# fgvieira/ngsF-HMM

Measured on AMD Instinct MI355X. Metric: site-ind updates/sec (EM iterations x individuals x sites / s), 1M sites x 1k ind, higher is better.
Workload: dtype f64

## Files before the change

ngsf-hmm_amd/csrc/kernels_fast.hip:

```cpp
#include <hip/hip_runtime.h>

#include "fast_dev.hpp"

namespace nghmm {

namespace {


__global__ void __launch_bounds__(256)
k_fast_geno_interleave(const uint32_t* __restrict__ codes, uint64_t cell0, uint64_t I, uint64_t S,
                       uint64_t T, uint32_t C, uint32_t* __restrict__ geno_il) {
  const uint64_t TB = T >> 4;
  const uint64_t n = I * C * TB * 64;
  for (uint64_t k = (uint64_t)blockIdx.x * blockDim.x + threadIdx.x; k < n;
       k += (uint64_t)gridDim.x * blockDim.x) {
    const uint64_t lane = k & 63, r = k >> 6;
    const uint64_t tb = r % TB, wv = r / TB;
    const uint64_t c = wv % C, i = wv / C;
    const uint64_t s0 = (c * 64 + lane) * T + tb * 16;
    uint32_t w = 0;
#pragma unroll
    for (int j = 0; j < 16; ++j) {
      const uint64_t s = s0 + j;
      if (s < S) w |= gl_code(codes, cell0 + s * I + i) << (2 * j);
// ... 150 lines not shown
      const uint32_t code = (w >> ((uint32_t)(t & 15) * 2)) & 3u;
      const double u = arr.u_lin;
      const double u0 = fma(u, h00, fma(u, 2 * bb, u * h02));
      const double u1 = fma(u, h00 + bb, u * (h02 + bb));
      e0 = code == 0 ? h00 : code == 1 ? 2 * bb : code == 2 ? h02 : u0;
      e1 = code == 0 ? h00 + bb : code == 1 ? 0.0 : code == 2 ? h02 + bb : u1;
    } else {
      const double* g = gl_lin + (s * I + i) * 3;
      e0 = fma(g[0], h00, fma(g[1], 2 * bb, g[2] * h02));
      e1 = fma(g[0], h00 + bb, g[2] * (h02 + bb));
    }
    out[k * 2] = log(e0);
    out[k * 2 + 1] = log(e1);
  }
}

struct SwitchName {
  const char* name;
  int Switches::*field;
};
const SwitchName kSwitches[] = {
    {"bg_parts", &Switches::bg_parts}, {"estmaf_interp", &Switches::estmaf_interp},
    {"estmaf_no_rows", &Switches::estmaf_no_rows}, {"estmaf_no_called", &Switches::estmaf_no_called},
    {"fast_c", &Switches::fast_c}, {"exact_serial", &Switches::exact_serial},
    {"dbg_abort_round", &Switches::dbg_abort_round}, {"no_dev_bfgs", &Switches::no_dev_bfgs},
    {"no_bg_stream", &Switches::no_bg_stream}, {"spans", &Switches::spans},
    {"viterbi_chunk", &Switches::viterbi_chunk}};

}

Switches Switches::from_env() {
  Switches sw;
  for (const auto& k : kSwitches) {
    std::string env = "NGHMM_";
    for (const char* c = k.name; *c; ++c) env += (char)std::toupper((unsigned char)*c);
    if (const char* v = std::getenv(env.c_str())) {
      char* end = nullptr;
      const long n = std::strtol(v, &end, 10);
      sw.*(k.field) = (end != v) ? (int)n : 1;
    }
  }
  return sw;
}

bool Switches::set(const char* name, long value) {
  for (const auto& k : kSwitches)
// ... 217 lines not shown
```

ngsf-hmm_amd/csrc/kernels_fast.hpp:

```cpp
#pragma once

#include <hip/hip_runtime.h>

#include <cstdint>
#include <map>
#include <vector>

#include "glview.hpp"

namespace nghmm {

struct Switches {
  int bg_parts = 2;
  int estmaf_interp = 1;
  int estmaf_no_rows = 0;
  int estmaf_no_called = 0;
  int fast_c = 0;
  int exact_serial = 0;
  int dbg_abort_round = 0;
  int no_dev_bfgs = 0;
  int no_bg_stream = 0;
  int viterbi_chunk = 0;
  int spans = 0;
  static Switches from_env();
  bool set(const char* name, long value);
};

struct SiteShard {
  uint32_t rank = 0, world = 1;
  double* send = nullptr;
  double* recv = nullptr;
  uint64_t cap = 0;
  int (*allgather)(void* user, uint64_t n_bytes) = nullptr;
  void* user = nullptr;
  double* edges = nullptr;
  bool edges_from_round = false;
  uint64_t n_gathers = 0;
};

// ... 58 lines not shown
    double *snap_F = nullptr, *snap_A = nullptr;
    uint32_t snap_set = 0;
    volatile uint32_t* h_table = nullptr;
    double *h_F = nullptr, *h_A = nullptr;
    unsigned long long stats_host[6] = {0, 0, 0, 0, 0, 0};
    uint32_t seq_base = 0;
    uint32_t mstep_no = 0;
    bool clean = true;
    bool preplanned = false;
    bool pre_F_fixed = false, pre_alpha_fixed = false;
    double* h_epi_lkl = nullptr;
    volatile uint32_t* h_epi = nullptr;
    uint32_t epi_seq = 0;
  } dev;

  double dmax_finite = 0;
  double alpha_small_min = 0;
  uint8_t* redo = nullptr;
  size_t redo_cap = 0;
  uint8_t* est_status = nullptr;
  double* est_state = nullptr;
  std::map<uint32_t, uint64_t> mode_ind_rounds;
  uint32_t* est_counts = nullptr;
};

enum EstCount {
  EST_CNT_CHECK_FAILED = 0,
  EST_CNT_RESUMED = 1,
  EST_CNT_RESUMED_AGAIN = 2,
  EST_CNT_LOGSPACE = 3,
  EST_CNT_EXACT_TAIL = 4,
  EST_COUNTS = 5
};

bool fast_create(FastState& fs, uint64_t I, uint64_t S, bool packed = false);
bool fast_create_replica(FastState& fs, const FastState& parent);
void fast_destroy(FastState& fs);
bool fast_load(FastState& fs, hipStream_t st, const GlView& gl_log, const double* d_pos);
bool fast_refresh_freq_table(FastState& fs, hipStream_t st, const double* d_freq, int* d_flags);
bool fast_refresh_emissions(FastState& fs, hipStream_t st, const double* d_freq, int* d_flags);
bool fast_lkl_prepare(FastState& fs, hipStream_t st, uint32_t n_pts, const uint32_t* h_ind,
                      const double* h_F, const double* h_A, bool force_general = false);
bool fast_lkl_launch(FastState& fs, hipStream_t st, double* d_lkl, int* d_flags,
                     bool emit_estep = false);
bool fast_lkl_covers_everyone(const FastState& fs);
bool dbfgs_available(const FastState& fs);
bool dbfgs_reserve(FastState& fs);
void dbfgs_destroy(FastState& fs);
void dbfgs_invalidate(FastState& fs);
constexpr uint32_t kEpiFlags = 8;
bool dbfgs_epilogue(FastState& fs, hipStream_t st, int* d_flags, uint32_t n_flags, const double* d_lkl);
bool dbfgs_wait_epilogue(FastState& fs, hipStream_t st, int* flags_out, uint32_t n_flags, bool yield);
bool dbfgs_begin(FastState& fs, hipStream_t st, double* d_indF, double* d_alpha, bool F_fixed,
                 bool alpha_fixed);
const double* dbfgs_start_F(const FastState& fs);
// ... 36 lines not shown
```

ngsf-hmm_amd/csrc/kernels_fast_estmaf.hip:

```cpp
#include "fast_dev.hpp"

#include <mutex>

namespace capi {
void set_error(const char* fmt, ...);
}

namespace nghmm {

namespace {



__device__ double2 estmaf_term_logspace(const double* g, double freq, double F) {
  double h[3];
  h[0] = (1 - freq) * (1 - freq) + (1 - freq) * freq * F;
  h[1] = 2 * (1 - freq) * freq - 2 * (1 - freq) * freq * F;
  h[2] = freq * freq + (1 - freq) * freq * F;
  double pp[3];
  for (int k = 0; k < 3; ++k) {
    double l = log(h[k]);
    if (l == -__builtin_huge_val()) l = -kINF;
    h[k] = l;
  }
// ... 69 lines not shown
    const int l = __builtin_amdgcn_update_dpp(0, (int)(uint32_t)b, 0x142, 0xa, 0xf, false);
    const int h = __builtin_amdgcn_update_dpp(0, (int)(uint32_t)(b >> 32), 0x142, 0xa, 0xf, false);
    v += ngh_from_bits(((uint64_t)(uint32_t)h << 32) | (uint32_t)l);
  }
  return v;
}

constexpr int EN = 12;
constexpr int EST_SCALARS = 8;
constexpr int EST_FIELDS = EST_SCALARS + 2 * EN;
enum : uint8_t { EST_DONE = 0, EST_INTERP = 1, EST_EXACT = 2 };
constexpr int EST_K0 = 2;
constexpr int EST_MIN_GAIN = 24;
constexpr double EST_DMAX = 0.85;
constexpr double EST_BACK = 0.1;
constexpr double EST_MULT = 32.0;
constexpr double EST_FIT = 0.72;
constexpr int EST_KMAX = 32;
constexpr double EST_TOL = 1e-11;
constexpr double EST_GUARD = 1e-9;
__constant__ double kChebC[EN] = {0.9914448613738104, 0.9238795325112867, 0.7933533402912352, 0.6087614290087207, 0.38268343236508984, 0.1305261922200517, -0.1305261922200516, -0.3826834323650895, -0.6087614290087207, -0.793353340291235, -0.9238795325112867, -0.9914448613738104};
__constant__ double kChebW[EN] = {0.13052619222005157, -0.3826834323650898, 0.6087614290087207, -0.7933533402912352, 0.9238795325112867, -0.9914448613738104, 0.9914448613738104, -0.9238795325112868, 0.7933533402912352, -0.6087614290087209, 0.3826834323650899, -0.130526192220052};

constexpr int ESTMAF_MAXW = 16;

__device__ __forceinline__ bool in_tile_rows(uint64_t site, uint64_t tile_T, uint64_t row0,
                                             uint64_t row1) {
  if (tile_T == 0) return true;
  const uint64_t j = site / tile_T, t = site - j * tile_T;
  const uint64_t row = (j >> 6) * tile_T + t;
  return row >= row0 && row < row1;
}
__host__ __device__ constexpr int estmaf_full_slots(int NI, int BLOCK) {
  return BLOCK == 64 ? (NI == 16 ? 12 : NI == 12 ? 8 : NI == 8 ? 4 : NI == 4 ? 2 : NI == 2 ? 1 : 0)
                     : (NI == 16 ? 8 : 0);
}

template <int NI, int BLOCK, bool TILE>
__device__ __forceinline__ void estmaf_site(
    const GlView& gl, const double* __restrict__ marg_blocks, uint64_t S_own, uint64_t I_tot,
    uint64_t I_blk, double* __restrict__ freq_out, uint8_t* __restrict__ redo,
    uint8_t* __restrict__ status, double* __restrict__ state, uint64_t state_stride, int fresh,
    int n_exact, int allow_build, uint64_t site, const double* __restrict__ tile_col,
    uint32_t* __restrict__ cnt, double (&xch)[2][ESTMAF_MAXW][2],
    double2 (&nodebuf)[(BLOCK == 64 && NI >= 8) ? EN : 1][(BLOCK == 64 && NI >= 8) ? 65 : 1],
    double2 (&xnode)[(BLOCK == 64 && NI >= 8) ? 1 : EN][(BLOCK == 64 && NI >= 8) ? 1 : BLOCK / 64],
    double2* park = nullptr) {
  constexpr int W = BLOCK / 64;
  constexpr bool PARK = (W == 1 && NI >= 8);
  const int lane = threadIdx.x & 63;
  const int wv = threadIdx.x >> 6;
  const uint32_t tix = threadIdx.x;
  constexpr uint64_t stride = BLOCK;
  const uint64_t cell_s = site * I_tot;

  double tF_lane_out;
  double sA[NI], sb[NI], sC[NI], u0[NI], nC[NI], fc[NI];
  {
    constexpr int NB = NI < 8 ? NI : (NI % 8 ? NI / 2 : 8);
    static_assert(NI % NB == 0, "whole batches");
    const bool one_block = (I_blk == I_tot);
    const uint32_t ib = (uint32_t)I_blk;
    double tF_acc = 0;
#pragma unroll
    for (int k0 = 0; k0 < NI; k0 += NB) {
      double r0[NB], r1[NB], r2[NB], rF[NB];
      uint64_t ic[NB];
// ... 254 lines not shown
                lane_sums(lane_value(r_nodes, nd), pn, pd);
                const double v = wave_sum_pair(pn, pd);
                const double sn = lane_value(v, 31), sd = lane_value(v, 63);
                if (lane == nd) {
                  an = sn;
                  ad = sd;
                }
              }
            }
            my_gn = an;
            my_gd = ad;
            check = true;
          }
        }
      }
    }
  }
  if (tix == 0) {
    const double freq = num / den;
    const bool ok = freq >= 0 && freq < 1;
    freq_out[site] = freq;
    redo[site] = ok ? 0 : 1;
    status[site] = EST_DONE;
  }
}

__device__ __forceinline__ const double* estmaf_tile_col(const double* marg_blocks, uint64_t site,
                                                         uint64_t tile_T, uint64_t I_tot) {
  const uint64_t j = site / tile_T, t = site - j * tile_T;
  return marg_blocks + post_lane_off((j >> 6) * tile_T + t, j & 63, I_tot);
}

#define ESTMAF_SHARED(NI, BLOCK)                                                              \
  constexpr bool PARK_ = ((BLOCK) == 64 && (NI) >= 8);                                         \
  __shared__ double xch[2][ESTMAF_MAXW][2];                       \
  __shared__ double2 nodebuf[PARK_ ? EN : 1][PARK_ ? 65 : 1];                                  \
  __shared__ double2 xnode[PARK_ ? 1 : EN][PARK_ ? 1 : (BLOCK) / 64]

template <int NI, int BLOCK, bool TILE>
__global__ void __launch_bounds__(BLOCK) __attribute__((amdgpu_waves_per_eu(2)))
k_fast_estmaf(const GlView gl, const double* __restrict__ marg_blocks,
              uint64_t S_own, uint64_t I_tot, uint64_t I_blk, uint64_t tile_T,
              double* __restrict__ freq_out, uint8_t* __restrict__ redo,
              uint8_t* __restrict__ status, double* __restrict__ state, uint64_t state_stride,
              int n_exact, int allow_build, uint64_t blk0, uint32_t* __restrict__ cnt) {
  ESTMAF_SHARED(NI, BLOCK);
  uint64_t site;
  const double* tile_col = nullptr;
  if constexpr (TILE) {
    const uint64_t b = blockIdx.x + blk0, x = b & 7, k = b >> 3;
    const uint64_t q = ((k >> 3) << 6) + (x << 3) + (k & 7);
    const uint64_t tile_row = q >> 6, l = q & 63;
    const uint64_t c = tile_row / tile_T, t = tile_row - c * tile_T;
    site = (c * 64 + l) * tile_T + t;
    if (site >= S_own) return;
    tile_col = marg_blocks + post_lane_off(tile_row, l, I_tot);
  } else {
    site = blockIdx.x;
  }
  extern __shared__ double2 park_mem[];
  estmaf_site<NI, BLOCK, TILE>(gl, marg_blocks, S_own, I_tot, I_blk, freq_out, redo, status, state,
                               state_stride, 1, n_exact, allow_build, site, tile_col, cnt, xch, nodebuf,
                               xnode, park_mem);
}

template <int NI, int BLOCK, bool TILE>
__global__ void __launch_bounds__(BLOCK) __attribute__((amdgpu_waves_per_eu(2)))
k_fast_estmaf_resume(const GlView gl, const double* __restrict__ marg_blocks,
                     uint64_t S_own, uint64_t I_tot, uint64_t I_blk, uint64_t tile_T,
                     double* __restrict__ freq_out, uint8_t* __restrict__ redo,
                     uint8_t* __restrict__ status, double* __restrict__ state,
                     uint64_t state_stride, int n_exact, int allow_build, uint64_t row0,
                     uint64_t row1, uint32_t* __restrict__ cnt, int cnt_slot) {
  ESTMAF_SHARED(NI, BLOCK);
  extern __shared__ double2 park_mem[];
  const int lane = threadIdx.x & 63;
  for (uint64_t base = (uint64_t)blockIdx.x * 64; base < S_own; base += (uint64_t)gridDim.x * 64) {
    const uint64_t s = base + lane;
    const bool need = s < S_own && in_tile_rows(s, TILE ? tile_T : 0, row0, row1) &&
                      status[s] == EST_EXACT;
    uint64_t mask = __ballot(need);
    if (mask && threadIdx.x == 0) atomicAdd(cnt + cnt_slot, (uint32_t)__popcll(mask));
    if constexpr (BLOCK > 64) __syncthreads();
    while (mask) {
      const uint64_t site = base + (uint64_t)__builtin_ctzll(mask);
      mask &= mask - 1;
      const double* tile_col = TILE ? estmaf_tile_col(marg_blocks, site, tile_T, I_tot) : nullptr;
      estmaf_site<NI, BLOCK, TILE>(gl, marg_blocks, S_own, I_tot, I_blk, freq_out, redo, status,
                                   state, state_stride, 0, n_exact, allow_build, site, tile_col, cnt,
                                   xch, nodebuf, xnode, park_mem);
      if constexpr (BLOCK > 64) __syncthreads();
    }
  }
}

__device__ __forceinline__ double row_sum(double v) {
  v = __dadd_rn(v, dpp_move<0xB1>(v));
  v = __dadd_rn(v, dpp_move<0x4E>(v));
  v = __dadd_rn(v, dpp_move<0x141>(v));
  v = __dadd_rn(v, dpp_move<0x140>(v));
  return v;
}

template <int NI, bool TILE>
__device__ __forceinline__ void estmaf_rows_sites(
    const GlView& gl, const double* __restrict__ marg_blocks, uint64_t S_own, uint64_t I_tot,
    uint64_t I_blk, double* __restrict__ freq_out, uint8_t* __restrict__ redo,
    uint8_t* __restrict__ status, double* __restrict__ state, uint64_t state_stride, int fresh,
    int n_exact, int allow_build, uint64_t site, const double* __restrict__ tile_col, bool done,
    uint32_t* __restrict__ cnt) {
  static_assert(EN <= 16, "a row's lanes hold the interval's node sums");
  const int lane = threadIdx.x, j = lane & 15;
  const uint64_t cell_s = site * I_tot;

  double sA[NI], sb[NI], sC[NI], u0[NI], nC[NI], fc[NI];
  double tF_acc = 0;
  {
    const bool one_block = (I_blk == I_tot);
    const uint32_t ib = (uint32_t)I_blk;
    double r0[NI], r1[NI], r2[NI], rF[NI];
    uint64_t ic[NI];
#pragma unroll
    for (int k = 0; k < NI; ++k) {
      const uint64_t i = (uint64_t)j + 16 * k;
      ic[k] = i < I_tot ? i : I_tot - 1;
      gl_fetch(gl, cell_s + ic[k], r0[k], r1[k], r2[k]);
    }
#pragma unroll
    for (int k = 0; k < NI; ++k) {
      if constexpr (TILE) {
        rF[k] = tile_col[post_ind_off(ic[k])];
      } else if (one_block) {
        rF[k] = marg_blocks[site * I_blk + ic[k]];
// ... 80 lines not shown
      const double bn = row_sum(q * my_gn) / Sq, bd = row_sum(q * my_gd) / Sq;
      if (check && !done) {
        interp_ok = fabs(bn - sn) <= EST_TOL * fabs(sn) && fabs(bd - sd) <= EST_TOL * fabs(sd);
        if (!interp_ok && j == 0) atomicAdd(cnt + EST_CNT_CHECK_FAILED, 1u);
      }
      check = false;
    }
    bool want_build = false;
    if (!done) {
      num = fma(r, sn, num);
      den = fma(r, sd, den + tF_sum);
      const double lhs = fabs(fma(pnum, den, -(num * pden))), thr = kEPS * (den * pden);
      const bool again = (lhs > thr) && (iters++ < 100);
      rprev = r;
      pnum = num;
      pden = den;
      if (!again) {
        if (j == 0) {
          const double freq = num / den;
          const bool ok = freq >= 0 && freq < 1;
          freq_out[site] = freq;
          redo[site] = ok ? 0 : 1;
          status[site] = EST_DONE;
        }
        done = true;
      } else if (interp_ok) {
        if (j < EN) {
          state[(EST_SCALARS + j) * state_stride + site] = my_gn;
          state[(EST_SCALARS + EN + j) * state_stride + site] = my_gd;
        }
        if (j == 0) {
          state[0 * state_stride + site] = num;
          state[1 * state_stride + site] = den;
          state[2 * state_stride + site] = pnum;
          state[3 * state_stride + site] = pden;
          state[4 * state_stride + site] = (double)iters;
          state[5 * state_stride + site] = mid;
          state[6 * state_stride + site] = half;
          state[7 * state_stride + site] = tF_sum;
          status[site] = EST_INTERP;
        }
        done = true;
      } else if (!built && --n_before <= 0) {
        const double m_est = (double)iters * (sqrt(lhs / thr) - 1.0);
        const double rn = pnum * rcp_nr2(pden - pnum);
        const double step = fabs(rn - rprev);
// ... 21 lines not shown
            want_build = true;
          }
        }
      }
    }
    if (__builtin_amdgcn_ballot_w64(want_build) != 0) {
#pragma unroll 1
      for (int nd = 0; nd < EN; ++nd) {
        const double tn = half * kChebC[nd];
        double qn, qd;
        lane_sums(mid * (1 + tn) * rcp_nr2(1 - tn), qn, qd);
        const double gn = row_sum(qn), gd = row_sum(qd);
        if (want_build && j == nd) {
          my_gn = gn;
          my_gd = gd;
        }
      }
      if (want_build) check = true;
    }
    if (__builtin_amdgcn_ballot_w64(!done) == 0) break;
  }
}

template <int NI, bool TILE>
__global__ void __launch_bounds__(64)
k_fast_estmaf_rows(const GlView gl, const double* __restrict__ marg_blocks, uint64_t S_own,
                   uint64_t I_tot, uint64_t I_blk, uint64_t tile_T, double* __restrict__ freq_out,
                   uint8_t* __restrict__ redo, uint8_t* __restrict__ status,
                   double* __restrict__ state, uint64_t state_stride, int n_exact,
                   int allow_build, uint32_t* __restrict__ cnt) {
  const int lane = threadIdx.x, row = lane >> 4;
  uint64_t site;
  const double* tile_col = nullptr;
  if constexpr (TILE) {
    const uint64_t b = blockIdx.x, x = b & 7, k = b >> 3;
    const uint64_t q = ((k >> 1) << 6) + (x << 3) + ((k & 1) << 2) + row;
    const uint64_t tile_row = q >> 6, l = q & 63;
    const uint64_t c = tile_row / tile_T, t = tile_row - c * tile_T;
    site = (c * 64 + l) * tile_T + t;
    tile_col = marg_blocks + post_lane_off(tile_row, l, I_tot);
  } else {
    site = (uint64_t)blockIdx.x * 4 + row;
  }
  bool done = site >= S_own;
  if (done) {
    site = 0;
    if constexpr (TILE) tile_col = marg_blocks;
  }
  if (__builtin_amdgcn_ballot_w64(!done) == 0) return;
  estmaf_rows_sites<NI, TILE>(gl, marg_blocks, S_own, I_tot, I_blk, freq_out, redo, status, state,
                              state_stride, 1, n_exact, allow_build, site, tile_col, done, cnt);
}

template <int NI, bool TILE>
__global__ void __launch_bounds__(64)
k_fast_estmaf_rows_resume(const GlView gl, const double* __restrict__ marg_blocks, uint64_t S_own,
                          uint64_t I_tot, uint64_t I_blk, uint64_t tile_T,
                          double* __restrict__ freq_out, uint8_t* __restrict__ redo,
                          uint8_t* __restrict__ status, double* __restrict__ state,
                          uint64_t state_stride, int n_exact, int allow_build,
                          uint32_t* __restrict__ cnt, int cnt_slot) {
  const int lane = threadIdx.x, row = lane >> 4;
  for (uint64_t base = (uint64_t)blockIdx.x * 64; base < S_own; base += (uint64_t)gridDim.x * 64) {
    const uint64_t s = base + lane;
    uint64_t mask = __ballot(s < S_own && status[s] == EST_EXACT);
    if (mask && lane == 0) atomicAdd(cnt + cnt_slot, (uint32_t)__popcll(mask));
    while (mask) {
      uint64_t site = 0;
      bool done = true;
#pragma unroll
      for (int r = 0; r < 4; ++r) {
        if (mask) {
          const uint64_t cand = base + (uint64_t)__builtin_ctzll(mask);
          mask &= mask - 1;
          if (r == row) {
            site = cand;
            done = false;
          }
        }
      }
      const double* tile_col =
          TILE ? (done ? marg_blocks : estmaf_tile_col(marg_blocks, site, tile_T, I_tot)) : nullptr;
      estmaf_rows_sites<NI, TILE>(gl, marg_blocks, S_own, I_tot, I_blk, freq_out, redo, status,
                                  state, state_stride, 0, n_exact, allow_build, site, tile_col, done,
                                  cnt);
    }
  }
}

__global__ void __launch_bounds__(256)
k_fast_estmaf_interp(uint64_t S_own, double* __restrict__ freq_out, uint8_t* __restrict__ redo,
                     uint8_t* __restrict__ status, double* __restrict__ state,
                     uint64_t state_stride, uint64_t tile_T, uint64_t row0, uint64_t row1) {
  const uint64_t site = (uint64_t)blockIdx.x * blockDim.x + threadIdx.x;
  if (site >= S_own || !in_tile_rows(site, tile_T, row0, row1) || status[site] != EST_INTERP)
    return;
  double num = state[0 * state_stride + site], den = state[1 * state_stride + site];
  double pnum = state[2 * state_stride + site], pden = state[3 * state_stride + site];
  int iters = (int)state[4 * state_stride + site];
  const double mid = state[5 * state_stride + site], half = state[6 * state_stride + site];
  const double tF_sum = state[7 * state_stride + site];
  double gn[EN], gd[EN];
#pragma unroll
  for (int j = 0; j < EN; ++j) {
    gn[j] = state[(EST_SCALARS + j) * state_stride + site];
    gd[j] = state[(EST_SCALARS + EN + j) * state_stride + site];
  }
  double cn[EN], cd[EN];
#pragma unroll
  for (int k = 0; k < EN; ++k) cn[k] = cd[k] = 0;
#pragma unroll
  for (int j = 0; j < EN; ++j) {
    const double x = kChebC[j], fn = gn[j] * (2.0 / EN), fd = gd[j] * (2.0 / EN);
    double t0 = 1.0, t1 = x;
    cn[0] += fn;
    cd[0] += fd;
#pragma unroll
    for (int k = 1; k < EN; ++k) {
      cn[k] = fma(fn, t1, cn[k]);
// ... 19 lines not shown
      bd2 = bd1;
      bd1 = bd0;
    }
    const double sn = fma(0.5 * x2, bn1, 0.5 * cn[0] - bn2);
    const double sd = fma(0.5 * x2, bd1, 0.5 * cd[0] - bd2);
    const double num2 = fma(r, sn, num), den2 = fma(r, sd, den + tF_sum);
    const double lhs = fabs(fma(pnum, den2, -(num2 * pden))), thr = kEPS * (den2 * pden);
    if (!(fabs(lhs - thr) >= EST_GUARD * thr)) break;
    num = num2;
    den = den2;
    const bool again = (lhs > thr) && (iters++ < 100);
    pnum = num;
    pden = den;
    if (!again) {
      st = EST_DONE;
      break;
    }
  }
  if (st == EST_DONE) {
    const double freq = num / den;
    const bool ok = freq >= 0 && freq < 1;
    freq_out[site] = freq;
    redo[site] = ok ? 0 : 1;
  } else {
    state[0 * state_stride + site] = num;
    state[1 * state_stride + site] = den;
    state[2 * state_stride + site] = pnum;
    state[3 * state_stride + site] = pden;
    state[4 * state_stride + site] = (double)iters;
  }
  status[site] = st;
}

constexpr int ESTC_A0 = 0, ESTC_B0 = 1, ESTC_M0 = 2, ESTC_M1 = 3, ESTC_M2 = 4;

template <bool TILE>
__global__ void __launch_bounds__(64)
k_fast_estmaf_called_sums(const GlView gl, const double* __restrict__ marg_blocks, uint64_t S_own,
                          uint64_t I_tot, uint64_t I_blk, uint64_t tile_T,
                          uint8_t* __restrict__ redo, double* __restrict__ state,
                          uint64_t state_stride, uint64_t blk0) {
  const int lane = threadIdx.x;
  uint64_t site;
  const double* tile_col = nullptr;
  if constexpr (TILE) {
    const uint64_t b = blockIdx.x + blk0, x = b & 7, k = b >> 3;
    const uint64_t q = ((k >> 3) << 6) + (x << 3) + (k & 7);
    const uint64_t tile_row = q >> 6, l = q & 63;
    const uint64_t c = tile_row / tile_T, t = tile_row - c * tile_T;
    site = (c * 64 + l) * tile_T + t;
    if (site >= S_own) return;
    tile_col = marg_blocks + post_lane_off(tile_row, l, I_tot);
  } else {
    site = blockIdx.x;
// ... 112 lines not shown
        pn += fma(w2, tF, w1) * inv;
        pd += fma(w0 + w2, tF, 2 * w1) * inv;
      } else {
        double lg[3] = {log(p0), log(p1), log(p2)};
        for (int k = 0; k < 3; ++k)
          if (lg[k] == -__builtin_huge_val()) lg[k] = -kINF;
        const double2 tt = estmaf_term_logspace(lg, freq, F);
        pn += tt.x;
        pd += tt.y;
      }
    }
    num += wave_sum(pn);
    den += wave_sum(pd);
    freq = num / den;
    again = (fabs(prev - freq) > kEPS) && (iters++ < 100);
  } while (again);
  if (lane == 0) freq_out[site] = freq;
}

__global__ void __launch_bounds__(256)
k_fast_estmaf_stream(const GlView gl, const double* __restrict__ marg_blocks,
                     uint64_t S_own, uint64_t I_tot, uint64_t I_blk, uint64_t tile_T,
                     double* __restrict__ freq_out, const uint8_t* __restrict__ redo,
                     uint64_t row0, uint64_t row1, uint32_t* __restrict__ cnt) {
  const int lane = threadIdx.x & 63;
  const uint64_t wave = (uint64_t)blockIdx.x * (blockDim.x >> 6) + (threadIdx.x >> 6);
  const uint64_t n_waves = (uint64_t)gridDim.x * (blockDim.x >> 6);
  if (!redo) {
    for (uint64_t site = wave; site < S_own; site += n_waves)
      if (in_tile_rows(site, tile_T, row0, row1))
        estmaf_stream_site(gl, marg_blocks, S_own, I_tot, I_blk, tile_T, freq_out, site, lane);
    return;
  }
  for (uint64_t base = wave * 64; base < S_own; base += n_waves * 64) {
    const uint64_t s = base + lane;
    const bool need = s < S_own && in_tile_rows(s, tile_T, row0, row1) && redo[s];
    uint64_t mask = __ballot(need);
    if (mask && lane == 0) atomicAdd(cnt + EST_CNT_LOGSPACE, (uint32_t)__popcll(mask));
    while (mask) {
      const int b = __builtin_ctzll(mask);
      mask &= mask - 1;
      estmaf_stream_site(gl, marg_blocks, S_own, I_tot, I_blk, tile_T, freq_out, base + b, lane);
    }
  }
}

}


bool fast_estmaf_called(const FastState& fs, const GlView& gl) {
  return !gl.dense && gl.codes && fs.called_table && !fs.sw.estmaf_no_called;
}

bool fast_estmaf_in_place(const FastState& fs, uint64_t I_tot) {
  return I_tot <= 8192 || (fs.packed && fs.called_table && !fs.sw.estmaf_no_called);
}

bool fast_estmaf_splittable(const FastState& fs, uint64_t I_tot, bool tile_major) {
  if (tile_major && fs.packed && fs.called_table && !fs.sw.estmaf_no_called) return true;
  return tile_major && I_tot > 128 && I_tot <= 8192;
}

bool fast_estmaf_reserve(FastState& fs, uint64_t S_own) {
  if (!fs.est_counts) {
    if (hipMalloc((void**)&fs.est_counts, EST_COUNTS * sizeof(uint32_t)) != hipSuccess) return false;
    if (hipMemset(fs.est_counts, 0, EST_COUNTS * sizeof(uint32_t)) != hipSuccess) return false;
    if (hipDeviceSynchronize() != hipSuccess) return false;
  }
  if (S_own <= fs.redo_cap) return true;
  if (fs.redo) (void)hipFree(fs.redo);
  if (fs.est_status) (void)hipFree(fs.est_status);
  if (fs.est_state) (void)hipFree(fs.est_state);
  fs.redo = fs.est_status = nullptr;
  fs.est_state = nullptr;
  fs.redo_cap = 0;
  if (hipMalloc((void**)&fs.redo, S_own) != hipSuccess) return false;
  if (hipMalloc((void**)&fs.est_status, S_own) != hipSuccess) return false;
  if (hipMalloc((void**)&fs.est_state, S_own * EST_FIELDS * sizeof(double)) != hipSuccess) return false;
  fs.redo_cap = S_own;
  return true;
}

static bool estmaf_dyn_lds(const void* kernel, size_t bytes) {
  if (bytes <= 65536) return true;
  static std::vector<std::pair<const void*, int>> told;
  static std::mutex mu;
  int dev = 0;
  (void)hipGetDevice(&dev);
  std::lock_guard<std::mutex> lock(mu);
// ... 23 lines not shown
  const uint64_t blk0 = row0 * 64, nblk = (row1 - row0) * 64;
  if (nblk == 0) return true;
  if (tile_major && !((I_tot <= 8192 || fast_estmaf_called(fs, d_gl_sites)) && I_blk == I_tot &&
                      S_own == fs.S))
    return false;
  const uint64_t tile_T = tile_major ? fs.T : 0;
  const bool stream_all = I_tot > 8192 && !tile_major;
  const uint64_t stream_wgs = stream_all ? (S_own + 3) / 4 : (S_own + 255) / 256;
  const dim3 grid((unsigned)(stream_wgs < 65536 ? stream_wgs : 65536)), block(256);
  if (!fast_estmaf_reserve(fs, S_own)) return false;
  if (fast_estmaf_called(fs, d_gl_sites)) {
    if (tile_major)
      hipLaunchKernelGGL((k_fast_estmaf_called_sums<true>), dim3((unsigned)nblk), dim3(64), 0, st,
                         d_gl_sites, d_marg_blocks, S_own, I_tot, I_blk, tile_T, fs.redo, fs.est_state,
                         fs.redo_cap, blk0);
    else
      hipLaunchKernelGGL((k_fast_estmaf_called_sums<false>), dim3((unsigned)S_own), dim3(64), 0, st,
                         d_gl_sites, d_marg_blocks, S_own, I_tot, I_blk, tile_T, fs.redo, fs.est_state,
                         fs.redo_cap, (uint64_t)0);
    hipLaunchKernelGGL(k_fast_estmaf_called_passes, dim3((unsigned)((S_own + 255) / 256)), dim3(256), 0,
                       st, S_own, d_freq_out, fs.redo, fs.est_status, fs.est_state, fs.redo_cap, tile_T,
                       row0, row1);
    hipLaunchKernelGGL(k_fast_estmaf_stream, grid, block, 0, st, d_gl_sites, d_marg_blocks, S_own,
                       I_tot, I_blk, tile_T, d_freq_out, fs.redo, row0, row1, fs.est_counts);
    return hipGetLastError() == hipSuccess;
  }
  bool interp = true;
  interp = fs.sw.estmaf_interp != 0;
  const uint64_t scan_wgs_all = (S_own + 63) / 64;
  const unsigned scan_wgs = (unsigned)(scan_wgs_all < 16384 ? scan_wgs_all : 16384);
#define ESTMAF_DYN(B) ((B) > 64 ? (size_t)EN * (B) * sizeof(double2) : (size_t)0)
#define ESTMAF_TELL(K, B) estmaf_dyn_lds(reinterpret_cast<const void*>(K), ESTMAF_DYN(B))
#define LAUNCH_NI(N, B)                                                                         \
  do {                                                                                          \
    if (fresh) {                                                                                \
      if (!ESTMAF_TELL((k_fast_estmaf<N, B, false>), B)) return false;                          \
      hipLaunchKernelGGL((k_fast_estmaf<N, B, false>), dim3((unsigned)S_own), dim3(B),          \
                         ESTMAF_DYN(B), st, d_gl_sites, d_marg_blocks, S_own, I_tot, I_blk,     \
                         (uint64_t)0, d_freq_out, fs.redo, fs.est_status, fs.est_state,         \
                         fs.redo_cap, n_exact, allow_build, (uint64_t)0, fs.est_counts);        \
    } else {                                                                                    \
      if (!ESTMAF_TELL((k_fast_estmaf_resume<N, B, false>), B)) return false;                   \
      hipLaunchKernelGGL((k_fast_estmaf_resume<N, B, false>), dim3(scan_wgs), dim3(B),          \
                         ESTMAF_DYN(B), st, d_gl_sites, d_marg_blocks, S_own, I_tot, I_blk,     \
                         (uint64_t)0, d_freq_out, fs.redo, fs.est_status, fs.est_state,         \
                         fs.redo_cap, n_exact, allow_build, row0, row1, fs.est_counts,          \
                         cnt_slot);                                                             \
    }                                                                                           \
  } while (0)
#define LAUNCH_TILE(N, B)                                                                       \
  do {                                                                                          \
    if (fresh) {                                                                                \
      if (!ESTMAF_TELL((k_fast_estmaf<N, B, true>), B)) return false;                           \
      hipLaunchKernelGGL((k_fast_estmaf<N, B, true>), dim3((unsigned)nblk), dim3(B),            \
                         ESTMAF_DYN(B), st, d_gl_sites, d_marg_blocks, S_own, I_tot, I_blk,     \
                         tile_T, d_freq_out, fs.redo, fs.est_status, fs.est_state, fs.redo_cap, \
                         n_exact, allow_build, blk0, fs.est_counts);                            \
    } else {                                                                                    \
      if (!ESTMAF_TELL((k_fast_estmaf_resume<N, B, true>), B)) return false;                    \
      hipLaunchKernelGGL((k_fast_estmaf_resume<N, B, true>), dim3(scan_wgs), dim3(B),           \
                         ESTMAF_DYN(B), st, d_gl_sites, d_marg_blocks, S_own, I_tot, I_blk,     \
                         tile_T, d_freq_out, fs.redo, fs.est_status, fs.est_state, fs.redo_cap, \
                         n_exact, allow_build, row0, row1, fs.est_counts, cnt_slot);            \
    }                                                                                           \
  } while (0)
#define LAUNCH_ROWS(N, TL)                                                                      \
  do {                                                                                          \
    if (fresh)                                                                                  \
      hipLaunchKernelGGL((k_fast_estmaf_rows<N, TL>),                                            \
                         dim3((unsigned)((TL) ? fs.Spad / 4 : (S_own + 3) / 4)), dim3(64), 0,   \
                         st, d_gl_sites, d_marg_blocks, S_own, I_tot, I_blk, tile_T, d_freq_out, \
                         fs.redo, fs.est_status, fs.est_state, fs.redo_cap, n_exact,            \
                         allow_build, fs.est_counts);                                           \
    else                                                                                        \
      hipLaunchKernelGGL((k_fast_estmaf_rows_resume<N, TL>), dim3(scan_wgs), dim3(64), 0, st,    \
                         d_gl_sites, d_marg_blocks, S_own, I_tot, I_blk, tile_T, d_freq_out,    \
                         fs.redo, fs.est_status, fs.est_state, fs.redo_cap, n_exact,            \
                         allow_build, fs.est_counts, cnt_slot);                                 \
  } while (0)
  const bool rows = I_tot <= 128 && !fs.sw.estmaf_no_rows;
  auto launch = [&](int fresh, int n_exact, int allow_build, int cnt_slot = 0) -> bool {
    if (rows) {
      if (tile_major) {
        if (I_tot <= 16) LAUNCH_ROWS(1, true);
        else if (I_tot <= 32) LAUNCH_ROWS(2, true);
        else if (I_tot <= 64) LAUNCH_ROWS(4, true);
        else LAUNCH_ROWS(8, true);
      } else {
        if (I_tot <= 16) LAUNCH_ROWS(1, false);
        else if (I_tot <= 32) LAUNCH_ROWS(2, false);
        else if (I_tot <= 64) LAUNCH_ROWS(4, false);
        else LAUNCH_ROWS(8, false);
      }
      return true;
    }
    if (tile_major) {
      if (I_tot <= 64) LAUNCH_TILE(1, 64);
      else if (I_tot <= 128) LAUNCH_TILE(2, 64);
      else if (I_tot <= 256) LAUNCH_TILE(4, 64);
      else if (I_tot <= 512) LAUNCH_TILE(8, 64);
      else if (I_tot <= 768) LAUNCH_TILE(12, 64);
      else if (I_tot <= 1024) LAUNCH_TILE(16, 64);
      else if (I_tot <= 1536) LAUNCH_TILE(12, 128);
      else if (I_tot <= 2048) LAUNCH_TILE(16, 128);
// ... 3 lines not shown
      else if (I_tot <= 6144) LAUNCH_TILE(12, 512);
      else if (I_tot <= 7168) LAUNCH_TILE(14, 512);
      else LAUNCH_TILE(16, 512);
    } else if (I_tot <= 64) LAUNCH_NI(1, 64);
    else if (I_tot <= 128) LAUNCH_NI(2, 64);
    else if (I_tot <= 256) LAUNCH_NI(4, 64);
    else if (I_tot <= 512) LAUNCH_NI(8, 64);
    else if (I_tot <= 768) LAUNCH_NI(12, 64);
    else if (I_tot <= 1024) LAUNCH_NI(16, 64);
    else if (I_tot <= 1536) LAUNCH_NI(12, 128);
    else if (I_tot <= 2048) LAUNCH_NI(16, 128);
    else if (I_tot <= 3072) LAUNCH_NI(12, 256);
    else if (I_tot <= 4096) LAUNCH_NI(16, 256);
    else if (I_tot <= 5120) LAUNCH_NI(10, 512);
    else if (I_tot <= 6144) LAUNCH_NI(12, 512);
    else if (I_tot <= 7168) LAUNCH_NI(14, 512);
    else LAUNCH_NI(16, 512);
    return true;
  };
  const uint8_t* redo = fs.redo;
  if (I_tot > 8192 && !tile_major) {
    redo = nullptr;
  } else if (!interp) {
    if (!launch(1, 0, 0)) return false;
  } else {
    const dim3 igrid((unsigned)((S_own + 255) / 256));
    if (!launch(1, EST_K0, 1)) return false;
    hipLaunchKernelGGL(k_fast_estmaf_interp, igrid, dim3(256), 0, st, S_own, d_freq_out, fs.redo,
                       fs.est_status, fs.est_state, fs.redo_cap, tile_T, row0, row1);
    for (int again = 0; again < 2; ++again) {
      if (!launch(0, 1, 1, again ? EST_CNT_RESUMED_AGAIN : EST_CNT_RESUMED)) return false;
      hipLaunchKernelGGL(k_fast_estmaf_interp, igrid, dim3(256), 0, st, S_own, d_freq_out, fs.redo,
                         fs.est_status, fs.est_state, fs.redo_cap, tile_T, row0, row1);
    }
    if (!launch(0, 0, 0, EST_CNT_EXACT_TAIL)) return false;
  }
  hipLaunchKernelGGL(k_fast_estmaf_stream, grid, block, 0, st, d_gl_sites, d_marg_blocks, S_own,
                     I_tot, I_blk, tile_T, d_freq_out, redo, row0, row1, fs.est_counts);
#undef LAUNCH_NI
#undef ESTMAF_DYN
#undef ESTMAF_TELL
#undef LAUNCH_TILE
#undef LAUNCH_ROWS
  return hipGetLastError() == hipSuccess;
}

}
```

Baseline: 42.27 billion.

## Gate estmaf follow-up kernels on device-side handoff counters to skip empty passes

```diff
diff --git a/ngsf-hmm_amd/csrc/kernels_fast.hip b/ngsf-hmm_amd/csrc/kernels_fast.hip
--- a/ngsf-hmm_amd/csrc/kernels_fast.hip
+++ b/ngsf-hmm_amd/csrc/kernels_fast.hip
@@ -196,6 +196,7 @@
 const SwitchName kSwitches[] = {
     {"bg_parts", &Switches::bg_parts}, {"estmaf_interp", &Switches::estmaf_interp},
     {"estmaf_no_rows", &Switches::estmaf_no_rows}, {"estmaf_no_called", &Switches::estmaf_no_called},
+    {"estmaf_no_fuse", &Switches::estmaf_no_fuse},
     {"fast_c", &Switches::fast_c}, {"exact_serial", &Switches::exact_serial},
     {"dbg_abort_round", &Switches::dbg_abort_round}, {"no_dev_bfgs", &Switches::no_dev_bfgs},
     {"no_bg_stream", &Switches::no_bg_stream}, {"spans", &Switches::spans},
diff --git a/ngsf-hmm_amd/csrc/kernels_fast.hpp b/ngsf-hmm_amd/csrc/kernels_fast.hpp
--- a/ngsf-hmm_amd/csrc/kernels_fast.hpp
+++ b/ngsf-hmm_amd/csrc/kernels_fast.hpp
@@ -15,6 +15,7 @@
   int estmaf_interp = 1;
   int estmaf_no_rows = 0;
   int estmaf_no_called = 0;
+  int estmaf_no_fuse = 0;
   int fast_c = 0;
   int exact_serial = 0;
   int dbg_abort_round = 0;
@@ -119,6 +120,7 @@
   double* est_state = nullptr;
   std::map<uint32_t, uint64_t> mode_ind_rounds;
   uint32_t* est_counts = nullptr;
+  uint32_t est_epoch = 0;
 };
 
 enum EstCount {
@@ -127,7 +129,13 @@
   EST_CNT_RESUMED_AGAIN = 2,
   EST_CNT_LOGSPACE = 3,
   EST_CNT_EXACT_TAIL = 4,
-  EST_COUNTS = 5
+  EST_COUNTS = 5,
+  EST_X_HAND0 = 5,
+  EST_X_HAND1 = 6,
+  EST_X_HAND2 = 7,
+  EST_X_REDO0 = 8,
+  EST_X_REDO1 = 9,
+  EST_COUNTS_ALLOC = 16
 };
 
 bool fast_create(FastState& fs, uint64_t I, uint64_t S, bool packed = false);
diff --git a/ngsf-hmm_amd/csrc/kernels_fast_estmaf.hip b/ngsf-hmm_amd/csrc/kernels_fast_estmaf.hip
--- a/ngsf-hmm_amd/csrc/kernels_fast_estmaf.hip
+++ b/ngsf-hmm_amd/csrc/kernels_fast_estmaf.hip
@@ -115,6 +115,19 @@
 __constant__ double kChebC[EN] = {0.9914448613738104, 0.9238795325112867, 0.7933533402912352, 0.6087614290087207, 0.38268343236508984, 0.1305261922200517, -0.1305261922200516, -0.3826834323650895, -0.6087614290087207, -0.793353340291235, -0.9238795325112867, -0.9914448613738104};
 __constant__ double kChebW[EN] = {0.13052619222005157, -0.3826834323650898, 0.6087614290087207, -0.7933533402912352, 0.9238795325112867, -0.9914448613738104, 0.9914448613738104, -0.9238795325112868, 0.7933533402912352, -0.6087614290087209, 0.3826834323650899, -0.130526192220052};
 
+struct EstGate {
+  uint32_t w;
+  static constexpr EstGate make(int hslot, int rslot, int gslot) {
+    return EstGate{(uint32_t)hslot << 4 | (uint32_t)rslot << 8 | (uint32_t)gslot << 12};
+  }
+  __device__ uint32_t* hcnt(uint32_t* cnt) const { return (w >> 4 & 15u) ? cnt + (w >> 4 & 15u) : nullptr; }
+  __device__ uint32_t* rcnt(uint32_t* cnt) const { return (w >> 8 & 15u) ? cnt + (w >> 8 & 15u) : nullptr; }
+  __device__ bool idle(const uint32_t* cnt) const {
+    const uint32_t g = w >> 12 & 15u;
+    return g && __hip_atomic_load(cnt + g, __ATOMIC_RELAXED, __HIP_MEMORY_SCOPE_AGENT) == 0;
+  }
+};
+
 constexpr int ESTMAF_MAXW = 16;
 
 __device__ __forceinline__ bool in_tile_rows(uint64_t site, uint64_t tile_T, uint64_t row0,
@@ -135,7 +148,7 @@
     uint64_t I_blk, double* __restrict__ freq_out, uint8_t* __restrict__ redo,
     uint8_t* __restrict__ status, double* __restrict__ state, uint64_t state_stride, int fresh,
     int n_exact, int allow_build, uint64_t site, const double* __restrict__ tile_col,
-    uint32_t* __restrict__ cnt, double (&xch)[2][ESTMAF_MAXW][2],
+    uint32_t* __restrict__ cnt, const EstGate fz, double (&xch)[2][ESTMAF_MAXW][2],
     double2 (&nodebuf)[(BLOCK == 64 && NI >= 8) ? EN : 1][(BLOCK == 64 && NI >= 8) ? 65 : 1],
     double2 (&xnode)[(BLOCK == 64 && NI >= 8) ? 1 : EN][(BLOCK == 64 && NI >= 8) ? 1 : BLOCK / 64],
     double2* park = nullptr) {
@@ -436,6 +449,7 @@
     freq_out[site] = freq;
     redo[site] = ok ? 0 : 1;
     status[site] = EST_DONE;
+    if (uint32_t* rc = ok ? nullptr : fz.rcnt(cnt)) atomicAdd(rc, 1u);
   }
 }
 
@@ -443,6 +457,16 @@
                                                          uint64_t tile_T, uint64_t I_tot) {
   const uint64_t j = site / tile_T, t = site - j * tile_T;
   return marg_blocks + post_lane_off((j >> 6) * tile_T + t, j & 63, I_tot);
+}
+
+__device__ __forceinline__ uint64_t estmaf_block_site(uint64_t b, uint64_t tile_T, uint64_t& tile_row,
+                                                      uint64_t& l) {
+  const uint64_t x = b & 7, k = b >> 3;
+  const uint64_t q = ((k >> 3) << 6) + (x << 3) + (k & 7);
+  tile_row = q >> 6;
+  l = q & 63;
+  const uint64_t c = tile_row / tile_T, t = tile_row - c * tile_T;
+  return (c * 64 + l) * tile_T + t;
 }
 
 #define ESTMAF_SHARED(NI, BLOCK)                                                              \
@@ -457,25 +481,24 @@
               uint64_t S_own, uint64_t I_tot, uint64_t I_blk, uint64_t tile_T,
               double* __restrict__ freq_out, uint8_t* __restrict__ redo,
               uint8_t* __restrict__ status, double* __restrict__ state, uint64_t state_stride,
-              int n_exact, int allow_build, uint64_t blk0, uint32_t* __restrict__ cnt) {
+              int n_exact, int allow_build, uint64_t blk0, uint32_t* __restrict__ cnt,
+              const EstGate fz) {
   ESTMAF_SHARED(NI, BLOCK);
   uint64_t site;
   const double* tile_col = nullptr;
+  const uint64_t b = blockIdx.x + (TILE ? blk0 : 0);
   if constexpr (TILE) {
-    const uint64_t b = blockIdx.x + blk0, x = b & 7, k = b >> 3;
-    const uint64_t q = ((k >> 3) << 6) + (x << 3) + (k & 7);
-    const uint64_t tile_row = q >> 6, l = q & 63;
-    const uint64_t c = tile_row / tile_T, t = tile_row - c * tile_T;
-    site = (c * 64 + l) * tile_T + t;
-    if (site >= S_own) return;
+    uint64_t tile_row, l;
+    site = estmaf_block_site(b, tile_T, tile_row, l);
     tile_col = marg_blocks + post_lane_off(tile_row, l, I_tot);
   } else {
-    site = blockIdx.x;
+    site = b;
   }
   extern __shared__ double2 park_mem[];
-  estmaf_site<NI, BLOCK, TILE>(gl, marg_blocks, S_own, I_tot, I_blk, freq_out, redo, status, state,
-                               state_stride, 1, n_exact, allow_build, site, tile_col, cnt, xch, nodebuf,
-                               xnode, park_mem);
+  if (site < S_own)
+    estmaf_site<NI, BLOCK, TILE>(gl, marg_blocks, S_own, I_tot, I_blk, freq_out, redo, status, state,
+                                 state_stride, 1, n_exact, allow_build, site, tile_col, cnt, fz,
+                                 xch, nodebuf, xnode, park_mem);
 }
 
 template <int NI, int BLOCK, bool TILE>
@@ -485,10 +508,11 @@
                      double* __restrict__ freq_out, uint8_t* __restrict__ redo,
                      uint8_t* __restrict__ status, double* __restrict__ state,
                      uint64_t state_stride, int n_exact, int allow_build, uint64_t row0,
-                     uint64_t row1, uint32_t* __restrict__ cnt, int cnt_slot) {
+                     uint64_t row1, uint32_t* __restrict__ cnt, int cnt_slot, const EstGate fz) {
   ESTMAF_SHARED(NI, BLOCK);
   extern __shared__ double2 park_mem[];
   const int lane = threadIdx.x & 63;
+  if (fz.idle(cnt)) return;
   for (uint64_t base = (uint64_t)blockIdx.x * 64; base < S_own; base += (uint64_t)gridDim.x * 64) {
     const uint64_t s = base + lane;
     const bool need = s < S_own && in_tile_rows(s, TILE ? tile_T : 0, row0, row1) &&
@@ -502,7 +526,7 @@
       const double* tile_col = TILE ? estmaf_tile_col(marg_blocks, site, tile_T, I_tot) : nullptr;
       estmaf_site<NI, BLOCK, TILE>(gl, marg_blocks, S_own, I_tot, I_blk, freq_out, redo, status,
                                    state, state_stride, 0, n_exact, allow_build, site, tile_col, cnt,
-                                   xch, nodebuf, xnode, park_mem);
+                                   fz, xch, nodebuf, xnode, park_mem);
       if constexpr (BLOCK > 64) __syncthreads();
     }
   }
@@ -522,7 +546,7 @@
     uint64_t I_blk, double* __restrict__ freq_out, uint8_t* __restrict__ redo,
     uint8_t* __restrict__ status, double* __restrict__ state, uint64_t state_stride, int fresh,
     int n_exact, int allow_build, uint64_t site, const double* __restrict__ tile_col, bool done,
-    uint32_t* __restrict__ cnt) {
+    uint32_t* __restrict__ cnt, const EstGate fz) {
   static_assert(EN <= 16, "a row's lanes hold the interval's node sums");
   const int lane = threadIdx.x, j = lane & 15;
   const uint64_t cell_s = site * I_tot;
@@ -649,6 +673,7 @@
           freq_out[site] = freq;
           redo[site] = ok ? 0 : 1;
           status[site] = EST_DONE;
+          if (uint32_t* rc = ok ? nullptr : fz.rcnt(cnt)) atomicAdd(rc, 1u);
         }
         done = true;
       } else if (interp_ok) {
@@ -716,22 +741,29 @@
   }
 }
 
+__device__ __forceinline__ uint64_t estmaf_rows_block_site(uint64_t b, uint64_t row, uint64_t tile_T,
+                                                           uint64_t& tile_row, uint64_t& l) {
+  const uint64_t x = b & 7, k = b >> 3;
+  const uint64_t q = ((k >> 1) << 6) + (x << 3) + ((k & 1) << 2) + row;
+  tile_row = q >> 6;
+  l = q & 63;
+  const uint64_t c = tile_row / tile_T, t = tile_row - c * tile_T;
+  return (c * 64 + l) * tile_T + t;
+}
+
 template <int NI, bool TILE>
 __global__ void __launch_bounds__(64)
 k_fast_estmaf_rows(const GlView gl, const double* __restrict__ marg_blocks, uint64_t S_own,
                    uint64_t I_tot, uint64_t I_blk, uint64_t tile_T, double* __restrict__ freq_out,
                    uint8_t* __restrict__ redo, uint8_t* __restrict__ status,
                    double* __restrict__ state, uint64_t state_stride, int n_exact,
-                   int allow_build, uint32_t* __restrict__ cnt) {
+                   int allow_build, uint32_t* __restrict__ cnt, const EstGate fz) {
   const int lane = threadIdx.x, row = lane >> 4;
   uint64_t site;
   const double* tile_col = nullptr;
   if constexpr (TILE) {
-    const uint64_t b = blockIdx.x, x = b & 7, k = b >> 3;
-    const uint64_t q = ((k >> 1) << 6) + (x << 3) + ((k & 1) << 2) + row;
-    const uint64_t tile_row = q >> 6, l = q & 63;
-    const uint64_t c = tile_row / tile_T, t = tile_row - c * tile_T;
-    site = (c * 64 + l) * tile_T + t;
+    uint64_t tile_row, l;
+    site = estmaf_rows_block_site(blockIdx.x, row, tile_T, tile_row, l);
     tile_col = marg_blocks + post_lane_off(tile_row, l, I_tot);
   } else {
     site = (uint64_t)blockIdx.x * 4 + row;
@@ -741,9 +773,10 @@
     site = 0;
     if constexpr (TILE) tile_col = marg_blocks;
   }
-  if (__builtin_amdgcn_ballot_w64(!done) == 0) return;
-  estmaf_rows_sites<NI, TILE>(gl, marg_blocks, S_own, I_tot, I_blk, freq_out, redo, status, state,
-                              state_stride, 1, n_exact, allow_build, site, tile_col, done, cnt);
+  if (__builtin_amdgcn_ballot_w64(!done) != 0)
+    estmaf_rows_sites<NI, TILE>(gl, marg_blocks, S_own, I_tot, I_blk, freq_out, redo, status, state,
+                                state_stride, 1, n_exact, allow_build, site, tile_col, done, cnt,
+                                fz);
 }
 
 template <int NI, bool TILE>
@@ -753,11 +786,13 @@
                           double* __restrict__ freq_out, uint8_t* __restrict__ redo,
                           uint8_t* __restrict__ status, double* __restrict__ state,
                           uint64_t state_stride, int n_exact, int allow_build,
-                          uint32_t* __restrict__ cnt, int cnt_slot) {
+                          uint32_t* __restrict__ cnt, int cnt_slot, const EstGate fz) {
   const int lane = threadIdx.x, row = lane >> 4;
+  if (fz.idle(cnt)) return;
   for (uint64_t base = (uint64_t)blockIdx.x * 64; base < S_own; base += (uint64_t)gridDim.x * 64) {
     const uint64_t s = base + lane;
-    uint64_t mask = __ballot(s < S_own && status[s] == EST_EXACT);
+    const bool need = s < S_own && status[s] == EST_EXACT;
+    uint64_t mask = __ballot(need);
     if (mask && lane == 0) atomicAdd(cnt + cnt_slot, (uint32_t)__popcll(mask));
     while (mask) {
       uint64_t site = 0;
@@ -777,18 +812,17 @@
           TILE ? (done ? marg_blocks : estmaf_tile_col(marg_blocks, site, tile_T, I_tot)) : nullptr;
       estmaf_rows_sites<NI, TILE>(gl, marg_blocks, S_own, I_tot, I_blk, freq_out, redo, status,
                                   state, state_stride, 0, n_exact, allow_build, site, tile_col, done,
-                                  cnt);
-    }
-  }
-}
-
-__global__ void __launch_bounds__(256)
-k_fast_estmaf_interp(uint64_t S_own, double* __restrict__ freq_out, uint8_t* __restrict__ redo,
-                     uint8_t* __restrict__ status, double* __restrict__ state,
-                     uint64_t state_stride, uint64_t tile_T, uint64_t row0, uint64_t row1) {
-  const uint64_t site = (uint64_t)blockIdx.x * blockDim.x + threadIdx.x;
-  if (site >= S_own || !in_tile_rows(site, tile_T, row0, row1) || status[site] != EST_INTERP)
-    return;
+                                  cnt, fz);
+    }
+  }
+}
+
+__device__ __forceinline__ void estmaf_interp_lane(uint64_t site, double* __restrict__ freq_out,
+                                                   uint8_t* __restrict__ redo,
+                                                   uint8_t* __restrict__ status,
+                                                   double* __restrict__ state,
+                                                   uint64_t state_stride, uint32_t* h_cnt,
+                                                   uint32_t* r_cnt) {
   double num = state[0 * state_stride + site], den = state[1 * state_stride + site];
   double pnum = state[2 * state_stride + site], pden = state[3 * state_stride + site];
   int iters = (int)state[4 * state_stride + site];
@@ -854,14 +888,28 @@
     const bool ok = freq >= 0 && freq < 1;
     freq_out[site] = freq;
     redo[site] = ok ? 0 : 1;
+    if (!ok && r_cnt) atomicAdd(r_cnt, 1u);
   } else {
     state[0 * state_stride + site] = num;
     state[1 * state_stride + site] = den;
     state[2 * state_stride + site] = pnum;
     state[3 * state_stride + site] = pden;
     state[4 * state_stride + site] = (double)iters;
+    if (h_cnt) atomicAdd(h_cnt, 1u);
   }
   status[site] = st;
+}
+
+__global__ void __launch_bounds__(256)
+k_fast_estmaf_interp(uint64_t S_own, double* __restrict__ freq_out, uint8_t* __restrict__ redo,
+                     uint8_t* __restrict__ status, double* __restrict__ state,
+                     uint64_t state_stride, uint64_t tile_T, uint64_t row0, uint64_t row1,
+                     uint32_t* __restrict__ cnt, const EstGate fz) {
+  if (fz.idle(cnt)) return;
+  const uint64_t site = (uint64_t)blockIdx.x * blockDim.x + threadIdx.x;
+  if (site >= S_own || !in_tile_rows(site, tile_T, row0, row1) || status[site] != EST_INTERP)
+    return;
+  estmaf_interp_lane(site, freq_out, redo, status, state, state_stride, fz.hcnt(cnt), fz.rcnt(cnt));
 }
 
 constexpr int ESTC_A0 = 0, ESTC_B0 = 1, ESTC_M0 = 2, ESTC_M1 = 3, ESTC_M2 = 4;
@@ -1020,8 +1068,14 @@
 k_fast_estmaf_stream(const GlView gl, const double* __restrict__ marg_blocks,
                      uint64_t S_own, uint64_t I_tot, uint64_t I_blk, uint64_t tile_T,
                      double* __restrict__ freq_out, const uint8_t* __restrict__ redo,
-                     uint64_t row0, uint64_t row1, uint32_t* __restrict__ cnt) {
+                     uint64_t row0, uint64_t row1, uint32_t* __restrict__ cnt, int gslot,
+                     uint32_t zero_slots) {
   const int lane = threadIdx.x & 63;
+  if (gslot >= 0) {
+    if (blockIdx.x == 0 && threadIdx.x < 32 && ((zero_slots >> threadIdx.x) & 1u))
+      __hip_atomic_store(cnt + threadIdx.x, 0u, __ATOMIC_RELAXED, __HIP_MEMORY_SCOPE_AGENT);
+    if (__hip_atomic_load(cnt + gslot, __ATOMIC_RELAXED, __HIP_MEMORY_SCOPE_AGENT) == 0) return;
+  }
   const uint64_t wave = (uint64_t)blockIdx.x * (blockDim.x >> 6) + (threadIdx.x >> 6);
   const uint64_t n_waves = (uint64_t)gridDim.x * (blockDim.x >> 6);
   if (!redo) {
@@ -1061,8 +1115,8 @@
 
 bool fast_estmaf_reserve(FastState& fs, uint64_t S_own) {
   if (!fs.est_counts) {
-    if (hipMalloc((void**)&fs.est_counts, EST_COUNTS * sizeof(uint32_t)) != hipSuccess) return false;
-    if (hipMemset(fs.est_counts, 0, EST_COUNTS * sizeof(uint32_t)) != hipSuccess) return false;
+    if (hipMalloc((void**)&fs.est_counts, EST_COUNTS_ALLOC * sizeof(uint32_t)) != hipSuccess) return false;
+    if (hipMemset(fs.est_counts, 0, EST_COUNTS_ALLOC * sizeof(uint32_t)) != hipSuccess) return false;
     if (hipDeviceSynchronize() != hipSuccess) return false;
   }
   if (S_own <= fs.redo_cap) return true;
@@ -1132,7 +1186,7 @@
                        st, S_own, d_freq_out, fs.redo, fs.est_status, fs.est_state, fs.redo_cap, tile_T,
                        row0, row1);
     hipLaunchKernelGGL(k_fast_estmaf_stream, grid, block, 0, st, d_gl_sites, d_marg_blocks, S_own,
-                       I_tot, I_blk, tile_T, d_freq_out, fs.redo, row0, row1, fs.est_counts);
+                       I_tot, I_blk, tile_T, d_freq_out, fs.redo, row0, row1, fs.est_counts, -1, 0u);
     return hipGetLastError() == hipSuccess;
   }
   bool interp = true;
@@ -1148,14 +1202,14 @@
       hipLaunchKernelGGL((k_fast_estmaf<N, B, false>), dim3((unsigned)S_own), dim3(B),          \
                          ESTMAF_DYN(B), st, d_gl_sites, d_marg_blocks, S_own, I_tot, I_blk,     \
                          (uint64_t)0, d_freq_out, fs.redo, fs.est_status, fs.est_state,         \
-                         fs.redo_cap, n_exact, allow_build, (uint64_t)0, fs.est_counts);        \
+                         fs.redo_cap, n_exact, allow_build, (uint64_t)0, fs.est_counts, fz);    \
     } else {                                                                                    \
       if (!ESTMAF_TELL((k_fast_estmaf_resume<N, B, false>), B)) return false;                   \
       hipLaunchKernelGGL((k_fast_estmaf_resume<N, B, false>), dim3(scan_wgs), dim3(B),          \
                          ESTMAF_DYN(B), st, d_gl_sites, d_marg_blocks, S_own, I_tot, I_blk,     \
                          (uint64_t)0, d_freq_out, fs.redo, fs.est_status, fs.est_state,         \
                          fs.redo_cap, n_exact, allow_build, row0, row1, fs.est_counts,          \
-                         cnt_slot);                                                             \
+                         cnt_slot, fz);                                                         \
     }                                                                                           \
   } while (0)
 #define LAUNCH_TILE(N, B)                                                                       \
@@ -1165,13 +1219,13 @@
       hipLaunchKernelGGL((k_fast_estmaf<N, B, true>), dim3((unsigned)nblk), dim3(B),            \
                          ESTMAF_DYN(B), st, d_gl_sites, d_marg_blocks, S_own, I_tot, I_blk,     \
                          tile_T, d_freq_out, fs.redo, fs.est_status, fs.est_state, fs.redo_cap, \
-                         n_exact, allow_build, blk0, fs.est_counts);                            \
+                         n_exact, allow_build, blk0, fs.est_counts, fz);                        \
     } else {                                                                                    \
       if (!ESTMAF_TELL((k_fast_estmaf_resume<N, B, true>), B)) return false;                    \
       hipLaunchKernelGGL((k_fast_estmaf_resume<N, B, true>), dim3(scan_wgs), dim3(B),           \
                          ESTMAF_DYN(B), st, d_gl_sites, d_marg_blocks, S_own, I_tot, I_blk,     \
                          tile_T, d_freq_out, fs.redo, fs.est_status, fs.est_state, fs.redo_cap, \
-                         n_exact, allow_build, row0, row1, fs.est_counts, cnt_slot);            \
+                         n_exact, allow_build, row0, row1, fs.est_counts, cnt_slot, fz);        \
     }                                                                                           \
   } while (0)
 #define LAUNCH_ROWS(N, TL)                                                                      \
@@ -1181,15 +1235,16 @@
                          dim3((unsigned)((TL) ? fs.Spad / 4 : (S_own + 3) / 4)), dim3(64), 0,   \
                          st, d_gl_sites, d_marg_blocks, S_own, I_tot, I_blk, tile_T, d_freq_out, \
                          fs.redo, fs.est_status, fs.est_state, fs.redo_cap, n_exact,            \
-                         allow_build, fs.est_counts);                                           \
+                         allow_build, fs.est_counts, fz);                                       \
     else                                                                                        \
       hipLaunchKernelGGL((k_fast_estmaf_rows_resume<N, TL>), dim3(scan_wgs), dim3(64), 0, st,    \
                          d_gl_sites, d_marg_blocks, S_own, I_tot, I_blk, tile_T, d_freq_out,    \
                          fs.redo, fs.est_status, fs.est_state, fs.redo_cap, n_exact,            \
-                         allow_build, fs.est_counts, cnt_slot);                                 \
+                         allow_build, fs.est_counts, cnt_slot, fz);                             \
   } while (0)
   const bool rows = I_tot <= 128 && !fs.sw.estmaf_no_rows;
-  auto launch = [&](int fresh, int n_exact, int allow_build, int cnt_slot = 0) -> bool {
+  const EstGate no_fuse = EstGate::make(0, 0, 0);
+  auto launch = [&](int fresh, int n_exact, int allow_build, int cnt_slot, const EstGate& fz) -> bool {
     if (rows) {
       if (tile_major) {
         if (I_tot <= 16) LAUNCH_ROWS(1, true);
@@ -1239,21 +1294,35 @@
   if (I_tot > 8192 && !tile_major) {
     redo = nullptr;
   } else if (!interp) {
-    if (!launch(1, 0, 0)) return false;
+    if (!launch(1, 0, 0, 0, no_fuse)) return false;
   } else {
+    const bool gated = !fs.sw.estmaf_no_fuse;
+    const int rslot = !gated ? 0 : (fs.est_epoch++ & 1u) ? EST_X_REDO1 : EST_X_REDO0;
+    const int hand[3] = {gated ? EST_X_HAND0 : 0, gated ? EST_X_HAND1 : 0, gated ? EST_X_HAND2 : 0};
     const dim3 igrid((unsigned)((S_own + 255) / 256));
-    if (!launch(1, EST_K0, 1)) return false;
+    if (!launch(1, EST_K0, 1, 0, EstGate::make(0, rslot, 0))) return false;
     hipLaunchKernelGGL(k_fast_estmaf_interp, igrid, dim3(256), 0, st, S_own, d_freq_out, fs.redo,
-                       fs.est_status, fs.est_state, fs.redo_cap, tile_T, row0, row1);
+                       fs.est_status, fs.est_state, fs.redo_cap, tile_T, row0, row1, fs.est_counts,
+                       EstGate::make(hand[0], rslot, 0));
     for (int again = 0; again < 2; ++again) {
-      if (!launch(0, 1, 1, again ? EST_CNT_RESUMED_AGAIN : EST_CNT_RESUMED)) return false;
+      if (!launch(0, 1, 1, again ? EST_CNT_RESUMED_AGAIN : EST_CNT_RESUMED,
+                  EstGate::make(0, rslot, hand[again])))
+        return false;
       hipLaunchKernelGGL(k_fast_estmaf_interp, igrid, dim3(256), 0, st, S_own, d_freq_out, fs.redo,
-                         fs.est_status, fs.est_state, fs.redo_cap, tile_T, row0, row1);
-    }
-    if (!launch(0, 0, 0, EST_CNT_EXACT_TAIL)) return false;
+                         fs.est_status, fs.est_state, fs.redo_cap, tile_T, row0, row1, fs.est_counts,
+                         EstGate::make(hand[again + 1], rslot, hand[again]));
+    }
+    if (!launch(0, 0, 0, EST_CNT_EXACT_TAIL, EstGate::make(0, rslot, hand[2]))) return false;
+    if (gated) {
+      const uint32_t zero = (1u << EST_X_HAND0) | (1u << EST_X_HAND1) | (1u << EST_X_HAND2) |
+                            (1u << (rslot == EST_X_REDO0 ? EST_X_REDO1 : EST_X_REDO0));
+      hipLaunchKernelGGL(k_fast_estmaf_stream, grid, block, 0, st, d_gl_sites, d_marg_blocks, S_own,
+                         I_tot, I_blk, tile_T, d_freq_out, redo, row0, row1, fs.est_counts, rslot, zero);
+      return hipGetLastError() == hipSuccess;
+    }
   }
   hipLaunchKernelGGL(k_fast_estmaf_stream, grid, block, 0, st, d_gl_sites, d_marg_blocks, S_own,
-                     I_tot, I_blk, tile_T, d_freq_out, redo, row0, row1, fs.est_counts);
+                     I_tot, I_blk, tile_T, d_freq_out, redo, row0, row1, fs.est_counts, -1, 0u);
 #undef LAUNCH_NI
 #undef ESTMAF_DYN
 #undef ESTMAF_TELL
```

After: 42.46 billion, median of 6. Within noise of the previous version (+0.4%).
